# AlvinHon/ring-zk

Hardware: AMD Instinct MI355X
Metric: proofs/sec (commit+challenge+response+verify), N=1024, batch=4096; NTT GB/s vs HBM peak (higher is better)
Workload: dtype u32

## Files before the change

### ring_zk_amd/csrc/rzk_core.h

```cpp
#pragma once
#include <stdint.h>

#if defined(__HIPCC__)
#include <hip/hip_runtime.h>
#define RZK_HD __host__ __device__ __forceinline__
#else
#define RZK_HD inline
#endif

namespace rzk {

constexpr int kMaxPrimes = 3;
constexpr int kKeyImages = kMaxPrimes;
constexpr int kTableLog = 12;
constexpr int kTableLen = 1 << kTableLog;

constexpr uint32_t kPrimes[kMaxPrimes] = {1073692673u, 1073668097u, 1073651713u};
constexpr uint32_t kPrimeGenerators[kMaxPrimes] = {3u, 3u, 10u};

struct PrimeConsts {
  uint32_t p;
  uint32_t twop;
  uint32_t npinv;
  uint32_t r2;
// ... 189 lines not shown
RZK_HD void inv_phase1(uint32_t* x, const uint32_t* tw, const PrimeConsts& pc) {
  using G = Geo<LOGN, LL>;
#pragma unroll
  for (int s = G::LE - 1; s >= 0; --s) {
    const int half = G::E >> (s + 1);
#pragma unroll
    for (int e = 0; e < G::E; ++e) {
      if (e & half) continue;
      const uint32_t w = tw[(1 << s) + (e >> (G::LE - s))];
      bfly_inv(x[e], x[e + half], w, pc);
    }
  }
}

RZK_HD uint32_t lift(int32_t v, const PrimeConsts& pc) { return (uint32_t)v + pc.twop; }

RZK_HD uint32_t mac_add(uint32_t acc, uint32_t x, uint32_t k, const PrimeConsts& pc) {
  return csub(acc + mont_lazy(x, k, pc.p, pc.npinv), pc.twop);
}
RZK_HD uint32_t mac_sub(uint32_t acc, uint32_t x, uint32_t k, const PrimeConsts& pc) {
  return csub(acc + pc.twop - mont_lazy(x, k, pc.p, pc.npinv), pc.twop);
}

struct CrtConsts {
  uint32_t q, qinv;
  uint32_t qhalf;
  uint32_t inv01_r;
  uint32_t p0_mod_p2_r;
  uint32_t inv012_r;
  uint32_t c1;
  uint32_t c2;
  uint32_t pmodq[4];
  uint32_t half1;
  uint32_t half3_d2;
  uint64_t half2;
  uint64_t half3_lo;
  uint32_t hmod[4][4];
  uint32_t hmodq[4];
  uint32_t r2q;
  uint32_t r48q;
};

RZK_HD int64_t montq(uint32_t a, uint32_t c, const CrtConsts& C) {
  uint64_t t = (uint64_t)a * c;
  uint32_t m = (uint32_t)t * C.qinv;
  uint32_t h = (uint32_t)(((uint64_t)m * C.q) >> 32);
  return (int64_t)(uint32_t)(t >> 32) - (int64_t)h;
}
template <int ROUNDS>
RZK_HD int64_t center_rounds(int64_t s, const CrtConsts& C) {
  const int64_t q = C.q, h = C.qhalf;
#pragma unroll
  for (int i = 0; i < ROUNDS; ++i) {
    s = s > h ? s - q : s;
    s = s < -h ? s + q : s;
  }
  return s;
}
RZK_HD int64_t crt_center(uint32_t r0, uint32_t r1, uint32_t r2, int np, const PrimeConsts* pc,
                          const CrtConsts& C) {
  const uint32_t d0 = csub(r0, pc[0].p);
  int64_t s = d0;
  bool neg;
// ... 37 lines not shown
  const uint32_t d = a - b;
  return a < b ? d + q : d;
}
RZK_HD uint32_t montq_u(uint32_t a, uint32_t c, const CrtConsts& C) {
  const uint64_t t = (uint64_t)a * c;
  const uint32_t m = (uint32_t)t * C.qinv;
  const uint32_t h = (uint32_t)(((uint64_t)m * C.q) >> 32);
  const uint32_t hi = (uint32_t)(t >> 32);
  const uint32_t d = hi - h;
  return hi < h ? d + C.q : d;
}
RZK_HD uint32_t zq_from_centered(int32_t a, uint32_t q) { return (uint32_t)a + (a < 0 ? q : 0u); }
RZK_HD int64_t center_from_zq(uint32_t u, const CrtConsts& C) {
  const uint32_t lo = u > C.qhalf ? u - C.q : u;
  return (int64_t)(int32_t)lo;
}
RZK_HD uint32_t crt2_zq(uint32_t r1, uint32_t d0, const PrimeConsts* pc, const CrtConsts& C) {
  const uint32_t t1 = r1 + pc[1].twop - d0;
  const uint32_t d1 = csub(mont_lazy(t1, C.inv01_r, pc[1].p, pc[1].npinv), pc[1].p);
  const uint32_t va = addq(d0, montq_u(d1, C.c1, C), C.q);
  const uint64_t x01 = (uint64_t)d1 * pc[0].p + d0;
  return subq(va, x01 >= C.half2 ? C.pmodq[2] : 0u, C.q);
}
RZK_HD uint32_t crt_digit1(uint32_t r, uint32_t d0, int np, const PrimeConsts* pc, const CrtConsts& C) {
  const uint32_t a1 = csub(csub(r + C.hmod[np][1], pc[1].twop), pc[1].p);
  const uint32_t t1 = a1 + pc[1].p - csub(d0, pc[1].p);
  return csub(mont_lazy(t1, C.inv01_r, pc[1].p, pc[1].npinv), pc[1].p);
}
RZK_HD uint32_t crt_value01_modq(uint32_t d0, uint32_t d1, const CrtConsts& C) {
  return addq(d0, montq_u(d1, C.c1, C), C.q);
}
RZK_HD uint32_t crt_value01_modp2(uint32_t d0, uint32_t d1, const PrimeConsts* pc, const CrtConsts& C) {
  const uint32_t m1 = mont_lazy(d1, C.p0_mod_p2_r, pc[2].p, pc[2].npinv);
  return csub(csub(d0, pc[2].p) + m1, pc[2].twop);
}
RZK_HD void crt_fold1(uint32_t r, int np, const PrimeConsts* pc, const CrtConsts& C, uint32_t& stA,
                      uint32_t& stB) {
  const uint32_t d0 = stA;
  const uint32_t d1 = crt_digit1(r, d0, np, pc, C);
  stA = crt_value01_modq(d0, d1, C);
  if (np == 3) stB = crt_value01_modp2(d0, d1, pc, C);
}
RZK_HD void crt_fold2(uint32_t r, const PrimeConsts* pc, const CrtConsts& C, uint32_t& stA, uint32_t stB) {
  const uint32_t a2 = csub(csub(r + C.hmod[3][2], pc[2].twop), pc[2].p);
  const uint32_t t2 = a2 + pc[2].twop - stB;
  const uint32_t d2 = csub(mont_lazy(t2, C.inv012_r, pc[2].p, pc[2].npinv), pc[2].p);
// ... 132 lines not shown
```

### ring_zk_amd/csrc/rzk_ctx.cpp

```cpp
#include "rzk_ctx.h"

namespace rzk::api {

void wipe(void* p, size_t n) {
  volatile uint8_t* v = (volatile uint8_t*)p;
  for (size_t i = 0; i < n; ++i) v[i] = 0;
}

int fail(rzk_ctx* c, int code, const char* msg) {
  if (c) c->err = msg;
  return code;
}

LaunchCfg cfg_of(rzk_ctx* c) {
  (void)hipSetDevice(c->device);
  return LaunchCfg{(void*)c->stream, c->num_cus, c->pair_poly ? 1 : 0, c->unit_io ? 1 : 0, c->shift_bytes ? 1 : 0};
}

int arena_reserve(rzk_ctx* c, Arena& a, size_t bytes) {
  if (bytes <= a.cap) return RZK_OK;
  HIPCHK(c, hipStreamSynchronize(c->stream));
  if (a.p) HIPCHK(c, hipFree(a.p));
  a.p = nullptr;
  a.cap = 0;
// ... 52 lines not shown
  constexpr Knob(const char* n, bool rzk_ctx::*f, const char* w) : name(n), kind(Bool), b(f), what(w) {}
  constexpr Knob(const char* n, Kind k, int rzk_ctx::*f, const char* w) : name(n), kind(k), i(f), what(w) {}
  constexpr Knob(const char* n, uint32_t rzk_ctx::*f, const char* w) : name(n), kind(Uint), u(f), what(w) {}
  constexpr Knob(const char* n, double rzk_ctx::*f, const char* w) : name(n), kind(Double), d(f), what(w) {}
};
const Knob kKnobs[] = {
    {"RZK_GRID_CUS", Knob::Clamped, &rzk_ctx::num_cus, "testing: CU count behind every grid cap and scratch size, in [1, the device's]"},
    {"RZK_SLOT_SHARE_MIN", &rzk_ctx::slot_share_min, "shared-operand path from this ratio of operand transforms to distinct operands"},
    {"RZK_ROW_GROUPS", &rzk_ctx::use_groups, "0: no row groups"},
    {"RZK_GROUP_MAX", Knob::Clamped, &rzk_ctx::group_max, "rows per group of row_group_kernel, in [1, the compiled accumulators]"},
    {"RZK_SHIFT", &rzk_ctx::use_shift, "0: challenge products as transforms, not rotations"},
    {"RZK_SHIFT_BYTES", &rzk_ctx::shift_bytes, "0: rotations of short operands as words, not packed bytes"},
    {"RZK_SUM_D", Knob::Flag, &rzk_ctx::sum_d, "Sum proof: force a2.(sum_i g_i v_i - v') on (1) or off (0); unset: by cost"},
    {"RZK_DKEY", Knob::Int, &rzk_ctx::use_dkey, "multiplier images: 0 never, 1 from kDkeyMinUses rows per multiplier on, 2 always"},
    {"RZK_LIN_E", &rzk_ctx::lin_e, "0: Linear verifier in the reference's grouping"},
    {"RZK_OIMG", &rzk_ctx::use_oimg, "0: Sum proof without operand images"},
    {"RZK_PRESET_IN_KERNEL", &rzk_ctx::preset_in_kernel, "0: verdict flags always preset by a fill launch"},
    {"RZK_PAIRS", &rzk_ctx::use_pairs, "0: unit_kernel without row pairs"},
    {"RZK_UPT", &rzk_ctx::units_per_task, "units per task of unit_kernel (0: automatic)"},
    {"RZK_VEC_ROWS", &rzk_ctx::vec_rows, "0: vector x vector programs on unit_kernel, not row_kernel"},
    {"RZK_PAIR_POLY", &rzk_ctx::pair_poly, "0: one wavefront per polynomial at N = 2048"},
    {"RZK_UNIT_IO", &rzk_ctx::unit_io, "0 / 1: force unit_kernel / unit_io_kernel for key-product programs (default: N = 512 only)"},
    {"RZK_BLOCK_MIN_LOGN", &rzk_ctx::block_min_logn, "row blocks from this log2 N on (12: never)"},
};

void read_knobs(rzk_ctx* c) {
  for (const Knob& k : kKnobs) {
    const char* e = std::getenv(k.name);
    if (!e) continue;
    switch (k.kind) {
      case Knob::Bool: c->*k.b = std::atoi(e) != 0; break;
      case Knob::Flag: c->*k.i = std::atoi(e) != 0 ? 1 : 0; break;
      case Knob::Int: c->*k.i = std::atoi(e); break;
      case Knob::Uint: c->*k.u = (uint32_t)std::atoi(e); break;
      case Knob::Double: c->*k.d = std::atof(e); break;
      case Knob::Clamped:
        if (k.i == &rzk_ctx::num_cus) {
          const long v = std::strtol(e, nullptr, 10);
          c->num_cus = v < 1 ? 1 : (v < c->num_cus ? (int)v : c->num_cus);
        } else {
          const int g = std::atoi(e);
          if (g >= 1 && g <= group_accumulators(c->logn)) c->group_max = g;
        }
        break;
    }
  }
// ... 26 lines not shown
  c->r2q = (uint32_t)((((unsigned __int128)1) << 64) % (unsigned __int128)q);
  c->n = n;
  c->k = k;
  c->l = l;
  c->kappa = kappa;
  c->b = b;
  c->sigma = b * (11ull * kappa) * isqrt_u64((uint64_t)k * N);
  c->commit_bound = 4 * c->sigma * isqrt_u64(N);
  c->verify_bound = 2 * c->sigma * isqrt_u64(N);
  if (!host::make_crt_consts((uint64_t)q, c->hT.crt)) {
    delete c;
    return create_fail(RZK_E_UNSUPPORTED, "modulus must be odd and below 4 * the smallest auxiliary prime");
  }
  if ((de = hipSetDevice(device)) != hipSuccess) {
    delete c;
    return create_fail(RZK_E_HIP, std::string("hipSetDevice: ") + hipGetErrorString(de));
  }
  hipDeviceProp_t prop;
  if (hipGetDeviceProperties(&prop, device) == hipSuccess && prop.multiProcessorCount > 0)
    c->num_cus = prop.multiProcessorCount;
  c->group_max = group_max_for((int)c->logn);
  c->unit_io = c->logn == 9;
  read_knobs(c);
  if ((de = hipStreamCreateWithFlags(&c->own_stream, hipStreamNonBlocking)) != hipSuccess) {
    delete c;
    return create_fail(RZK_E_HIP, std::string("hipStreamCreate: ") + hipGetErrorString(de));
  }
  c->stream = c->own_stream;

  std::vector<uint32_t> all((size_t)2 * kMaxPrimes * kTableLen);
  for (int i = 0; i < kMaxPrimes; ++i) {
    std::vector<uint32_t> f, v;
    host::make_twiddles(i, f, v);
    std::memcpy(&all[(size_t)(2 * i) * kTableLen], f.data(), sizeof(uint32_t) * kTableLen);
    std::memcpy(&all[(size_t)(2 * i + 1) * kTableLen], v.data(), sizeof(uint32_t) * kTableLen);
    c->hT.pc[i] = host::make_prime_consts(i, N);
  }
  bool okk = hipMalloc((void**)&c->d_tw, all.size() * sizeof(uint32_t)) == hipSuccess &&
             hipMemcpy(c->d_tw, all.data(), all.size() * sizeof(uint32_t), hipMemcpyHostToDevice) == hipSuccess;
  c->hT.cap[0] = 0.0;
  for (int np = 1; np <= kMaxPrimes; ++np) c->hT.cap[np] = host::crt_capacity(np);
  okk = okk && (c->small || hipMalloc((void**)&c->d_row_scratch,
                                      row_scratch_words((int)c->logn, c->num_cus) * sizeof(uint32_t)) == hipSuccess);
  okk = okk && hipMalloc((void**)&c->dT, sizeof(DevTables)) == hipSuccess &&
        hipMemcpy(c->dT, &c->hT, sizeof(DevTables), hipMemcpyHostToDevice) == hipSuccess;
  okk = okk && hipMalloc((void**)&c->d_bad, sizeof(uint32_t)) == hipSuccess &&
// ... 167 lines not shown
```

### ring_zk_amd/csrc/rzk_ctx.h

```cpp
#pragma once
#include <hip/hip_runtime.h>

#include <cmath>
#include <cstddef>
#include <cstdio>
#include <cstdlib>
#include <cstring>
#include <map>
#include <memory>
#include <string>
#include <utility>
#include <vector>

#include "../../include/rzk.h"
#include "rzk_chacha.h"
#include "rzk_core.h"
#include "rzk_dev.h"
#include "rzk_dgauss.h"
#include "rzk_keccak.h"
#include "rzk_packed.h"
#include "rzk_plan.h"
#include "rzk_reject.h"
#include "rzk_tables.h"
#include "rzk_xof.h"
// ... 31 lines not shown
struct rzk_ctx {
  int device = 0;
  hipStream_t own_stream = nullptr;
  hipStream_t stream = nullptr;
  int num_cus = 256;
  int64_t q = 0;
  uint32_t N = 0, logn = 0, n = 0, k = 0, l = 0, kappa = 0;
  uint64_t b = 0;
  uint64_t sigma = 0, commit_bound = 0, verify_bound = 0;
  DevTables hT{};
  DevTables* dT = nullptr;
  uint32_t* d_tw = nullptr;
  uint32_t* d_row_scratch = nullptr;
  uint32_t* d_group_scratch = nullptr;
  uint32_t* d_block_scratch = nullptr;
  uint32_t block_min_logn = 11;
  bool use_groups = true;
  uint32_t units_per_task = 0;
  bool vec_rows = true;
  bool unit_io = false;
  bool pair_poly = true;
  bool trusted = false;
  bool use_pairs = true;
  int group_max = 1;
  bool use_shift = true;
  bool shift_bytes = true;
  int use_dkey = 1;
  Arena ws_dkey;
  const uint32_t* dkey_img = nullptr;
  const double* dkey_l2 = nullptr;
  uint32_t dkey_n = 0;
  bool use_oimg = true;
  Arena ws_oimg;
  Operands oimg_state{};
  uint32_t oimg_producer_op = 0xffu;
  bool lin_e = true;
  int sum_d = -1;
  bool preset_in_kernel = true;
  bool small = false;
  uint32_t r2q = 0;
  uint32_t* d_key_mont = nullptr;
  bool key_loaded = false;
  std::vector<uint8_t> key_class;
  std::vector<int32_t> key_entry;
  uint32_t n_general = 0;
  uint32_t* d_key_ntt = nullptr;
// ... 135 lines not shown
```

### ring_zk_amd/csrc/rzk_dev.h

```cpp
#pragma once
#include <stddef.h>
#include <stdint.h>

#include <string>

#include "rzk_core.h"
#include "rzk_packed.h"
#include "rzk_wire_walk.h"

namespace rzk {

struct DevTables {
  PrimeConsts pc[kMaxPrimes];
  CrtConsts crt;
  double cap[kMaxPrimes + 1];
};

#if defined(__HIPCC__)
template <class Tp>
__device__ __forceinline__ Tp table_load(const Tp* p) {
#if defined(__HIP_DEVICE_COMPILE__)
  typedef const Tp __attribute__((address_space(4))) * cptr_t;
  return *reinterpret_cast<cptr_t>(reinterpret_cast<uintptr_t>(p));
#else
  return *p;
#endif
}
#endif
constexpr int kMaxOperands = 12;
constexpr int kMaxRows = 48;
constexpr int kMaxTerms = 640;
constexpr int kMaxAdds = 128;

enum : uint8_t { TERM_KEY = 0, TERM_VEC = 1, TERM_SHIFT = 2, TERM_DKEY = 3, TERM_DD = 4, TERM_KIND_MASK = 0x3f };
enum : uint8_t { MODE_STORE = 0, MODE_ZERO = 1 };
constexpr uint8_t TERM_CHECK = 0x80;
constexpr uint8_t TERM_CHECK2 = 0x40;
constexpr uint8_t ADD_CHECK = 0x80;
// ... 12 lines not shown
  uint16_t off;
};
struct alignas(8) Row {
  uint16_t term0, nterms, add0, nadds;
  uint8_t out_op, mode;
  uint16_t out_off;
  uint16_t nshift, pad;
};
constexpr int kGroupMax = 4;
struct GroupDesc {
  uint16_t row0, count;
};
struct Program {
  uint32_t nrows, nterms, nadds, ngroups;
  GroupDesc groups[kMaxRows];
  Row rows[kMaxRows];
  Term terms[kMaxTerms];
  AddTerm adds[kMaxAdds];
};

enum : uint8_t { ITEM_KEY = 0, ITEM_VEC = 1 };
constexpr uint16_t kNoKey = 0xffff;
constexpr uint16_t kNoRow = 0xffff;
struct alignas(8) Item {
  uint8_t kind;
  uint8_t flags;
  uint8_t b_op, a_op;
  uint16_t b_off, a_off;
  uint16_t keyA, keyB;
  int8_t signA, signB;
  uint16_t pad;
};
struct alignas(8) Unit {
  uint16_t rowA, rowB;
  uint16_t item0, nitems;
};
struct WaveProgram {
  uint32_t nunits, nitems;
  Unit units[kMaxRows];
  Item items[kMaxTerms];
};

constexpr int kMaxSlots = 512;
struct SlotTable {
  uint32_t nslots, pad;
  uint16_t op[kMaxSlots], off[kMaxSlots];
// ... 167 lines not shown
```

### ring_zk_amd/csrc/rzk_plan.h

```cpp
#pragma once
#include <cstring>
#include <map>
#include <utility>

#include "rzk_dev.h"

namespace rzk {

static_assert(sizeof(Term) == 8 && sizeof(AddTerm) == 4 && sizeof(Row) == 16 && sizeof(Item) == 16 && sizeof(Unit) == 8,
              "program record sizes");
static_assert(offsetof(Program, rows) % 8 == 0 && offsetof(Program, terms) % 8 == 0 && offsetof(Program, adds) % 4 == 0 &&
                  offsetof(WaveProgram, units) % 8 == 0 && offsetof(WaveProgram, items) % 8 == 0,
              "program record alignment");

enum KeyClass : uint8_t { KC_ZERO = 0, KC_ONE = 1, KC_GENERAL = 2 };

enum ProgId : int {
  PG_MATVEC = 0,
  PG_POLYMUL,
  PG_CMUL,
  PG_OPEN_COMMIT,
  PG_RESPONSE,
  PG_A1_RELATION,
  PG_LIN_COMMIT2,
// ... 14 lines not shown
  PG_LIN_V2B,
};

constexpr uint32_t kDkeyVar = 0x10000u;
constexpr uint32_t kOimgVar = 0x20000u;
constexpr uint32_t kRecoverVar = 0x40000u;
inline bool recover_capable(int id) {
  return id == PG_A1_RELATION || id == PG_REL_ROT || id == PG_LIN_V1B || id == PG_LIN_V2B || id == PG_SUM_V3 || id == PG_SUM_V4;
}

constexpr int kPlanOk = 0, kPlanArg = -1, kPlanUnsupported = -4;

struct PlanEnv {
  uint32_t n, k, l, logn;
  bool small;
  bool rot;
  uint32_t block_min_logn;
  bool use_groups;
  int group_max;
  bool use_pairs;
  double slot_share_min;
  const uint8_t* key_class;
  const int32_t* key_entry;
};

struct PlanFacts {
  uint32_t nrows = 0;
  uint32_t nunits = 0;
  uint32_t work = 0;
  bool has_vec = false;
  uint32_t nslots = 0;
  uint32_t np_store = 0;
  uint32_t ngroups = 0;
  uint32_t nblocks = 0;
  bool has_dkey = false;
  bool has_dd = false;
  bool shift = false;
  bool has_shift = false;
  bool two_bit = false;
  uint16_t polys_in[kMaxOperands] = {};
  uint32_t polys_out = 0;
};

struct Plan {
  Program prog;
  WaveProgram wave;
// ... 370 lines not shown
  uint32_t ng = 0;
  for (uint32_t r = 0; r < p.nrows;) {
    uint32_t cnt = 1;
    const Row& r0 = p.rows[r];
    while (cnt < gmax && r + cnt < p.nrows) {
      const Row& rr = p.rows[r + cnt];
      bool same = rr.nterms == r0.nterms && r0.nterms > 0;
      for (uint32_t t = 0; same && t < r0.nterms; ++t) {
        const Term& a = p.terms[r0.term0 + t];
        const Term& b2 = p.terms[rr.term0 + t];
        same = a.b_op == b2.b_op && a.b_off == b2.b_off;
      }
      if (!same) break;
      ++cnt;
    }
    p.groups[ng].row0 = (uint16_t)r;
    p.groups[ng].count = (uint16_t)cnt;
    ++ng;
    r += cnt;
  }
  return ng * 2 <= p.nrows ? ng : 0;
}

inline uint32_t plan_units(const Program& p, bool use_pairs, WaveProgram& wp) {
  auto key_only = [&](const Row& rr) {
    for (uint32_t t = 0; t < rr.nterms; ++t)
      if (kind_of(p.terms[rr.term0 + t]) != TERM_KEY) return false;
    return true;
  };
  uint32_t work = 0;
  for (uint32_t r = 0; r < p.nrows;) {
    const Row& ra = p.rows[r];
    Unit& un = wp.units[wp.nunits++];
    un.rowA = (uint16_t)r;
    un.rowB = kNoRow;
    un.item0 = (uint16_t)wp.nitems;
    un.nitems = ra.nterms;
    for (uint32_t t = 0; t < ra.nterms; ++t) {
      const Term& tm = p.terms[ra.term0 + t];
      Item& im = wp.items[wp.nitems++];
      im.kind = kind_of(tm) == TERM_VEC ? ITEM_VEC : ITEM_KEY;
      im.flags = tm.kind & (TERM_CHECK | TERM_CHECK2);
      im.b_op = tm.b_op;
      im.b_off = tm.b_off;
      im.a_op = tm.a_op;
      im.a_off = tm.a_off;
      im.keyA = im.kind == ITEM_KEY ? tm.a_off : 0;
      im.keyB = kNoKey;
      im.signA = tm.sign;
      im.signB = 0;
    }
    uint32_t step = 1;
    if (use_pairs && r + 1 < p.nrows && ra.nterms >= 1 && ra.nshift == 0 && key_only(ra)) {
      const Row& rb = p.rows[r + 1];
      if (rb.nterms == 1 && rb.nshift == 0 && key_only(rb)) {
        const Term& tb = p.terms[rb.term0];
        const Term& ta = p.terms[ra.term0 + ra.nterms - 1];
        if (tb.b_op == ta.b_op && tb.b_off == ta.b_off) {
          Item& im = wp.items[wp.nitems - 1];
          im.keyB = tb.a_off;
          im.signB = tb.sign;
          im.flags |= tb.kind & (TERM_CHECK | TERM_CHECK2);
          un.rowB = (uint16_t)(r + 1);
          step = 2;
        }
      }
    }
    work += (un.nitems ? un.nitems : 1u) + (un.rowB != kNoRow ? 2u : 1u);
    r += step;
  }
  return work;
}

inline bool plan_slots(const Program& p, double share_min, SlotTable& st) {
  std::map<OpOff, uint32_t> index;
  bool fits = true;
  uint32_t transforms = 0;
  auto slot_of = [&](uint8_t op, uint16_t off) -> uint32_t {
    auto it = index.find({op, off});
    if (it != index.end()) return it->second;
    if (st.nslots >= (uint32_t)kMaxSlots) { fits = false; return 0; }
    const uint32_t sidx = st.nslots++;
    st.op[sidx] = op;
    st.off[sidx] = off;
    index[{op, off}] = sidx;
    return sidx;
  };
  for (uint32_t t = 0; t < p.nterms; ++t) {
    const Term& tm = p.terms[t];
    const uint32_t sb = slot_of(tm.b_op, tm.b_off);
// ... 48 lines not shown
  bool key_only = p.nterms > 0, all_sparse = p.nterms > 0;
  for (uint32_t t = 0; t < p.nterms; ++t) {
    const Term& tm = p.terms[t];
    const uint8_t kind = kind_of(tm);
    key_only = key_only && kind == TERM_KEY;
    all_sparse = all_sparse && tm.kind == TERM_VEC && ((pb.sparse_ops >> tm.a_op) & 1u);
    f.has_vec = f.has_vec || kind == TERM_VEC;
    f.has_shift = f.has_shift || kind == TERM_SHIFT;
    f.has_dd = f.has_dd || kind == TERM_DD;
    f.has_dkey = f.has_dkey || kind == TERM_DKEY || kind == TERM_DD;
  }
  f.shift = env.rot && pb.sparse_ops && all_sparse;
  f.two_bit = pb.two_bit;
  f.nrows = p.nrows;
  if (!env.small && env.logn >= 10 && env.logn >= env.block_min_logn && !f.shift && !f.has_shift && !f.two_bit &&
      !f.has_dkey && p.nterms > 0) {
    plan.use_blocks = plan_blocks(p, key_only, plan.blocks);
    if (plan.use_blocks) f.nblocks = plan.blocks.nblocks;
  }
  if (!env.small && env.use_groups && !f.shift && !f.two_bit && !f.nblocks && !f.has_dkey && key_only)
    p.ngroups = f.ngroups = plan_groups(p, (uint32_t)env.group_max);
  if (!env.small) {
    plan.use_wave = true;
    f.work = plan_units(p, env.use_pairs, plan.wave);
    f.nunits = plan.wave.nunits;
  }
  if (!env.small && env.slot_share_min > 0 && p.nterms > 0 && f.ngroups == 0 && !f.shift && !f.has_shift &&
      !f.two_bit && !f.nblocks && !f.has_dkey) {
    plan.use_slots = plan_slots(p, env.slot_share_min, plan.slots);
    if (plan.use_slots) {
      f.nslots = plan.slots.nslots;
      f.np_store = f.has_vec ? 3 : 2;
    }
  }
  count_traffic(p, f);
  return kPlanOk;
}

}
```

### ring_zk_amd/csrc/rzk_rowprog.h

```cpp
#pragma once
#include "rzk_wave.h"

namespace rzk {

__device__ __forceinline__ int32_t canon_lo(int64_t c, uint32_t qhalf, uint32_t& bad) {
  bad |= (uint32_t)(((uint64_t)c + qhalf) >> 32);
  return (int32_t)c;
}
__device__ __forceinline__ int32_t canon_lo_mx(int64_t c, uint32_t qhalf, uint32_t& bad, uint32_t& mx) {
  const uint64_t s = (uint64_t)c + qhalf;
  bad |= (uint32_t)(s >> 32);
  const uint32_t lo = (uint32_t)s;
  mx = lo > mx ? lo : mx;
  return (int32_t)c;
}
__device__ __forceinline__ void canon_pair(const longlong2 t, uint32_t qhalf, uint32_t& bad, uint32_t& mx, int32_t& lo0,
                                           int32_t& lo1) {
  lo0 = canon_lo_mx(t.x, qhalf, bad, mx);
  lo1 = canon_lo_mx(t.y, qhalf, bad, mx);
}
__device__ __forceinline__ bool canon_fail(uint32_t bad, uint32_t mx, uint32_t qhalf) {
  return __any((bad != 0) | (mx > 2u * qhalf)) != 0;
}
__device__ __forceinline__ void input_fault(const Operands& ops, uint8_t* flags, uint32_t bo, int lane) {
// ... 234 lines not shown
      for (int i = 0; i < H; ++i) {
        const int64_t c = p[i * S::LANES + lane];
        vh[i] = canon ? canon_lo_mx(c, qhalf, bad, mx) : (int32_t)c;
      }
    }
    if (measure) {
#pragma unroll
      for (int i = 0; i < H; ++i) {
        const uint32_t uu = (uint32_t)vh[i];
        const uint32_t vv = vh[i] < 0 ? 0u - uu : uu;
        maxabs = vv > maxabs ? vv : maxabs;
      }
    }
    int32_t* base = ext + S::lane_base(lane) + h * HOFF;
#pragma unroll
    for (int i = 0; i < H; ++i) {
      const int32_t a = shift_part(vh[i], part);
      base[S::N + S::off(i)] = a;
      base[S::off(i)] = -a;
    }
  }
}

template <int LOGN, bool PAIR, bool TO_MEM, class TM = WaveTeam>
__device__ __forceinline__ void shift_product(uint32_t* res, bool fresh, bool minus, const int32_t* a,
                                              const int64_t* __restrict__ pv, int lane_in, int32_t* ext,
                                              const DevTables& T, bool& fault, bool trusted) {
  constexpr int LL = TM::LL;
  int lane = lane_in;
  if (LL != 6) asm volatile("" : "+v"(lane));
  using S = ShiftGeo<LOGN, PAIR, LL>;
  constexpr int E = S::E;
  constexpr int HW = TO_MEM ? (LL == 6 ? kShiftHMem : kShiftHMemPair) : kShiftH;
  constexpr int H = HW < E ? HW : E;
  constexpr int NCH = E / H;
  constexpr bool LIST = LL != 6;
  const uint32_t q = T.crt.q, qhalf = T.crt.qhalf;
  uint32_t vbad = 0, vmx = 0, maxv = 0;
  TM::sync();
  shift_fill_from<LOGN, PAIR, LL>(pv, lane, ext, SHIFT_WHOLE, true, !trusted, qhalf, vbad, vmx, maxv);
  if (!trusted) fault = fault || canon_fail(vbad, vmx, qhalf);
  uint64_t suma = 0;
#pragma unroll
  for (int i = 0; i < E; ++i) {
    const uint32_t ua = (uint32_t)a[i];
    suma += a[i] < 0 ? 0u - ua : ua;
  }
  const double bound = (double)TM::sum_u56(suma) * (double)TM::max_u32(maxv);
  const int npass = __builtin_amdgcn_readfirstlane(bound < 4.0e18 ? 1 : 2);
  int32_t* list = ext + S::WORDS;
  uint32_t lbase = 0, ltotal = 1;
  if (LIST) {
    const uint32_t mine = shift_count_nonzeros<E>(a);
    const uint32_t w = (uint32_t)__builtin_amdgcn_readfirstlane(lane >> 6);
    if ((lane & 63) == 0) list[2 * kShiftListCap + w] = (int32_t)mine;
    TM::sync();
// ... 382 lines not shown
```

### ring_zk_amd/csrc/rzk_run.cpp

```cpp
#include "rzk_ctx.h"

namespace rzk::api {

bool shift_ok(const rzk_ctx* c) { return c->use_shift && !c->small && (c->logn <= 10 || c->pair_poly); }

namespace {

PlanEnv plan_env(const rzk_ctx* c) {
  return PlanEnv{c->n, c->k, c->l, c->logn, c->small, shift_ok(c), c->block_min_logn, c->use_groups, c->group_max,
                 c->use_pairs, c->slot_share_min, c->key_class.data(), c->key_entry.data()};
}

template <class T>
int upload(rzk_ctx* c, const T* host, T** dev) {
  HIPCHK(c, hipMalloc((void**)dev, sizeof(T)));
  HIPCHK(c, hipMemcpyAsync(*dev, host, sizeof(T), hipMemcpyHostToDevice, c->stream));
  HIPCHK(c, hipStreamSynchronize(c->stream));
  return RZK_OK;
}

void free_program(DevProg& dp) {
  if (dp.d) (void)hipFree(dp.d);
  if (dp.d_slots) (void)hipFree(dp.d_slots);
  if (dp.d_blocks) (void)hipFree(dp.d_blocks);
  if (dp.d_wp) (void)hipFree(dp.d_wp);
}

int get_program(rzk_ctx* c, int id, uint32_t var, DevProg& out) {
  const bool needs_key = !(id == PG_POLYMUL || id == PG_CMUL || id == PG_RESPONSE || id == PG_SUM_XP ||
                           id == PG_SUM_W2 || id == PG_REL_ROT);
  if (needs_key && !c->key_loaded) return fail(c, RZK_E_STATE, "commitment key not loaded");
  auto it = c->progs.find({id, var});
  if (it != c->progs.end()) {
// ... 286 lines not shown
```

### ring_zk_amd/csrc/rzk_tables.h

```cpp
#pragma once
#include <cstdint>
#include <vector>

#include "rzk_core.h"

namespace rzk {
namespace host {

typedef unsigned __int128 u128;

inline uint64_t mulmod(uint64_t a, uint64_t b, uint64_t m) { return (uint64_t)((u128)a * b % m); }
inline uint64_t powmod(uint64_t b, uint64_t e, uint64_t m) {
  uint64_t r = 1 % m;
  b %= m;
  while (e) {
    if (e & 1) r = mulmod(r, b, m);
    b = mulmod(b, b, m);
    e >>= 1;
  }
  return r;
}
inline uint64_t invmod_prime(uint64_t a, uint64_t p) { return powmod(a, p - 2, p); }
inline uint32_t inv_u32(uint32_t odd) {
  uint32_t x = odd;
// ... 60 lines not shown
  C.p0_mod_p2_r = to_mont(p0 % p2, (uint32_t)p2);
  C.inv012_r = to_mont(invmod_prime(mulmod(p0 % p2, p1 % p2, p2), p2), (uint32_t)p2);
  C.c1 = (uint32_t)(((u128)(p0 % q) << 32) % q);
  C.c2 = (uint32_t)(((u128)mulmod(p0 % q, p1 % q, q) << 32) % q);
  C.pmodq[0] = 1 % q;
  C.pmodq[1] = (uint32_t)(p0 % q);
  C.pmodq[2] = (uint32_t)mulmod(p0 % q, p1 % q, q);
  C.pmodq[3] = (uint32_t)mulmod(C.pmodq[2], p2 % q, q);
  C.half1 = (uint32_t)((p0 + 1) / 2);
  C.half2 = (p0 * p1 + 1) / 2;
  const u128 P3 = (u128)p0 * p1 * p2;
  const u128 h3 = (P3 + 1) / 2;
  C.half3_d2 = (uint32_t)(h3 / (p0 * p1));
  C.half3_lo = (uint64_t)(h3 % (p0 * p1));
  for (int np = 0; np <= kMaxPrimes; ++np) {
    u128 P = 1;
    for (int i = 0; i < np; ++i) P *= kPrimes[i];
    const u128 H = (P - 1) / 2;
    for (int i = 0; i < 4; ++i) C.hmod[np][i] = i < kMaxPrimes ? (uint32_t)(H % kPrimes[i]) : 0;
    C.hmodq[np] = (uint32_t)(H % q);
  }
  C.r2q = (uint32_t)((((u128)1) << 64) % q);
  C.r48q = (uint32_t)((((u128)1) << 48) % q);
  return true;
}

inline double crt_capacity(int np) {
  long double P = 1;
  for (int i = 0; i < np; ++i) P *= (long double)kPrimes[i];
  return (double)((P - 1) / 2 * (1.0L - 1e-12L));
}

}
}
```

### ring_zk_amd/csrc/rzk_unit.h

```cpp
#pragma once
#include "rzk_rowprog.h"

namespace rzk {

constexpr int kScratchLines = 6;
#ifndef RZK_STAMPS
#define RZK_STAMPS 0
#endif
#if RZK_STAMPS
#define RZK_T0() const uint64_t t_sec0 = __builtin_amdgcn_s_memtime()
#define RZK_T1(acc) acc += __builtin_amdgcn_s_memtime() - t_sec0
#else
#define RZK_T0() do { } while (0)
#define RZK_T1(acc) do { } while (0)
#endif

__device__ __forceinline__ void set_priority_level(uint32_t level) {
  if (level == 0) __builtin_amdgcn_s_setprio(3);
  else if (level == 1) __builtin_amdgcn_s_setprio(2);
  else if (level == 2) __builtin_amdgcn_s_setprio(1);
  else __builtin_amdgcn_s_setprio(0);
}
__device__ __forceinline__ void set_progress_priority(uint32_t done, uint32_t total) {
  set_priority_level(__builtin_amdgcn_readfirstlane(total ? (done * 4u) / total : 0u));
// ... 69 lines not shown
  }
  if (!EARLY && pi == 2) {
#pragma unroll
    for (int g = 0; g < E / 4; ++g) sb[g] = B4[G::own4(li, g)];
  }
  if (pi == 0) {
    if (np == 1) {
#pragma unroll
      for (int e = 0; e < E; ++e) acc[e] = crt1_zq(acc[e], T.pc, T.crt);
      return true;
    }
    if (np == 2) {
#pragma unroll
      for (int e = 0; e < E; ++e) acc[e] = crt2_digit0(acc[e], T.pc);
    } else {
#pragma unroll
      for (int e = 0; e < E; ++e) acc[e] = crt_fold0(acc[e], np, T.pc, T.crt);
    }
#pragma unroll
    for (int g = 0; g < E / 4; ++g) A4[G::own4(li, g)] = make_uint4(acc[4 * g], acc[4 * g + 1], acc[4 * g + 2], acc[4 * g + 3]);
    return false;
  }
  if (pi == 1 && np == 2) {
#pragma unroll
    for (int g = 0; g < E / 4; ++g) {
      const uint4 dv = sa[g];
      const uint32_t d0[4] = {dv.x, dv.y, dv.z, dv.w};
#pragma unroll
      for (int i = 0; i < 4; ++i) acc[4 * g + i] = crt2_zq(acc[4 * g + i], d0[i], T.pc, T.crt);
    }
    return true;
  }
  if (pi == 1) {
#pragma unroll
    for (int g = 0; g < E / 4; ++g) {
      const uint4 dv = sa[g];
      const uint32_t d0[4] = {dv.x, dv.y, dv.z, dv.w};
      uint32_t va[4], vb[4];
#pragma unroll
      for (int i = 0; i < 4; ++i) {
        const uint32_t d1 = crt_digit1(acc[4 * g + i], d0[i], np, T.pc, T.crt);
        va[i] = crt_value01_modq(d0[i], d1, T.crt);
        vb[i] = crt_value01_modp2(d0[i], d1, T.pc, T.crt);
      }
      A4[G::own4(li, g)] = make_uint4(va[0], va[1], va[2], va[3]);
      B4[G::own4(li, g)] = make_uint4(vb[0], vb[1], vb[2], vb[3]);
// ... 91 lines not shown
#define RZK_STEP_PRIORITY()                             \
  do {                                                  \
    set_progress_priority(work_done, work_total);       \
    ++work_done;                                        \
  } while (0)

  for (uint32_t task = first_task; task < ntasks; task += gridDim.x * WPB) {
    const uint32_t b = task / tasks_per_entry;
    const uint32_t u0 = (task - b * tasks_per_entry) * units_per_task;
    const uint32_t u1 = u0 + units_per_task < nunits ? u0 + units_per_task : nunits;
    const uint32_t bo = ops.group > 1 ? b / ops.group : b;
    if (ops.preset) {
      if (lane == 0) flags[bo] = (uint8_t)ops.preset;
      if (TM::LL != 6) TM::sync();
    }
#pragma unroll 1
    for (uint32_t ui = u0; ui < u1; ++ui) {
      const Unit un = table_load(&wp->units[ui]);
      const Row rowA = table_load(&prog->rows[un.rowA]);
      const bool pair = un.rowB != kNoRow;
      const uint32_t un_items = un.nitems;
      const bool null_unit = un_items == 0;
      const bool has_shift = HAS_SHIFT && rowA.nshift > 0;
      if (has_shift) {
        bool fault = false;
        RZK_T0();
#pragma unroll 1
        for (uint32_t t = 0; t < rowA.nshift; ++t) {
          const Term tm = table_load(&prog->terms[rowA.term0 + rowA.nterms + t]);
          const int64_t* __restrict__ pa = operand_ptr(ops, tm.a_op, tm.a_off, b, bo, N);
          int32_t a[E];
          if (trusted) {
#pragma unroll
            for (int e = 0; e < E; ++e) a[e] = (int32_t)pa[G::j_p1(lane, e)];
          } else {
            uint32_t abad = 0, amx = 0;
#pragma unroll
            for (int e = 0; e < E; ++e) a[e] = canon_lo_mx(pa[G::j_p1(lane, e)], qhalf, abad, amx);
            fault = fault || canon_fail(abad, amx, qhalf);
          }
          shift_product<LOGN, false, true, TM>(st_sh, t == 0, tm.sign < 0, a, operand_ptr(ops, tm.b_op, tm.b_off, b, bo, N), lane,
                                           reinterpret_cast<int32_t*>(lds), T, fault, trusted);
        }
        if (fault) input_fault(ops, flags, bo, lane);
        TM::sync();
        RZK_T1(t_rot);
      }
// ... 9 lines not shown
#pragma unroll 1
        for (uint32_t it = 0; it < nit; ++it) {
          const bool last = it + 1 == nit;
          RZK_STEP_PRIORITY();
          int ln = lane;
          RZK_OPAQUE(ln);
          uint32_t acc[E];
#pragma unroll
          for (int c = 0; c < E; ++c) acc[c] = 0;
          if (!null_unit) {
            const Item im = table_load(&wp->items[un.item0 + it]);
            uint32_t x[E];
            float nb = 0.f;
            bool below = true;
            const bool chk = first && (im.flags & (TERM_CHECK | TERM_CHECK2));
            {
              RZK_T0();
              load_lift<LOGN, TM>(x, operand_ptr(ops, im.b_op, im.b_off, b, bo, N), ln, pc, first, nb, chk, ops.norm_limit, below, qhalf,
                              trusted, fault);
              RZK_T1(t_load);
            }
            if (chk && !below && (lane & 63) == 0) fail_check(flags + bo, ops.pad != 0, (im.flags & TERM_CHECK2) != 0);
            const bool vec = HAS_VEC && im.kind == ITEM_VEC;
            constexpr bool EARLY = E <= 16 && !HAS_VEC;
            uint32_t kreg[E];
            const uint4* __restrict__ kpA = reinterpret_cast<const uint4*>(key_ntt + ((size_t)im.keyA * kKeyImages + pi) * N);
            if (EARLY && !vec && im.keyA != kNoKey) {
#pragma unroll
              for (int g = 0; g < E / 4; ++g) {
                const uint4 kv = kpA[G::key4(ln, g)];
                kreg[4 * g] = kv.x, kreg[4 * g + 1] = kv.y, kreg[4 * g + 2] = kv.z, kreg[4 * g + 3] = kv.w;
              }
            }
            {
              RZK_T0();
              wave_fwd<LOGN, TM>(x, ln, lds, twf, pc);
              RZK_T1(t_fwd);
            }
            if (!EARLY && !vec && im.keyA != kNoKey) {
#pragma unroll
              for (int g = 0; g < E / 4; ++g) {
                const uint4 kv = kpA[G::key4(ln, g)];
                kreg[4 * g] = kv.x, kreg[4 * g + 1] = kv.y, kreg[4 * g + 2] = kv.z, kreg[4 * g + 3] = kv.w;
              }
            }
            uint32_t xb[E];
            if (vec) {
#pragma unroll
              for (int c = 0; c < E; ++c) xb[c] = csub(mont_lazy(x[c], pc.ninv_r2, pc.p, pc.npinv), pc.p);
              float na = 0.f;
              bool unused_below = true;
              load_lift<LOGN, TM>(x, operand_ptr(ops, im.a_op, im.a_off, b, bo, N), ln, pc, first, na, false, 0, unused_below, qhalf,
                              trusted, fault);
              wave_fwd<LOGN, TM>(x, ln, lds, twf, pc);
              if (first) boundA = bound_fma(na, nb, boundA);
            } else if (first) {
              if (im.keyA != kNoKey) boundA = bound_fma((float)key_l2[im.keyA], nb, boundA);
              if (pair && im.keyB != kNoKey) boundB = bound_fma((float)key_l2[im.keyB], nb, boundB);
            }
            const bool feedsA = vec || im.keyA != kNoKey;
            if (!last) {
              RZK_T0();
              if (vec) mac_park<LOGN, false, TM>(x, xb, im.signA < 0, P4, ln, it == 0, pc);
              else if (feedsA) mac_park<LOGN, false, TM>(x, kreg, im.signA < 0, P4, ln, it == 0, pc);
              RZK_T1(t_mac);
              continue;
            }
            RZK_T0();
            if (fault) input_fault(ops, flags, bo, lane);
            if (first) np = primes_for(boundA > boundB ? boundA : boundB, T);
#pragma unroll
            for (int c = 0; c < E; ++c) acc[c] = x[c];
            if (vec) {
              mac_park<LOGN, true, TM>(acc, xb, im.signA < 0, P4, ln, it == 0, pc);
            } else if (feedsA) {
              mac_park<LOGN, true, TM>(acc, kreg, im.signA < 0, P4, ln, it == 0, pc);
            } else {
#pragma unroll
              for (int g = 0; g < E / 4; ++g) {
                const uint4 v = P4[G::own4(ln, g)];
                acc[4 * g] = v.x, acc[4 * g + 1] = v.y, acc[4 * g + 2] = v.z, acc[4 * g + 3] = v.w;
              }
            }
            if (pair) {
              const uint4* __restrict__ kb = reinterpret_cast<const uint4*>(key_ntt + ((size_t)im.keyB * kKeyImages + pi) * N);
              uint32_t kbr[E];
#pragma unroll
              for (int g = 0; g < E / 4; ++g) {
                const uint4 kv = kb[G::key4(ln, g)];
                kbr[4 * g] = kv.x, kbr[4 * g + 1] = kv.y, kbr[4 * g + 2] = kv.z, kbr[4 * g + 3] = kv.w;
              }
              mac_park<LOGN, false, TM>(x, kbr, im.signB < 0, P4, ln, true, pc);
            }
            RZK_T1(t_mac);
          }
#pragma unroll 1
          for (uint32_t r = 0; r < (pair ? 2u : 1u); ++r) {
            if (r == 1) {
#pragma unroll
              for (int g = 0; g < E / 4; ++g) {
                const uint4 v = P4[G::own4(ln, g)];
                acc[4 * g] = v.x, acc[4 * g + 1] = v.y, acc[4 * g + 2] = v.z, acc[4 * g + 3] = v.w;
              }
            }
            bool done = true;
            RZK_STEP_PRIORITY();
            if (!null_unit) {
              RZK_T0();
              done = inverse_fold_global<LOGN, OPQ, TM>(pi, np, acc, lane, lds, twf + kTableLen, pc, st + (size_t)(2 * r) * N,
                                                    st + (size_t)(2 * r + 1) * N, T);
              RZK_T1(t_inv);
            }
            if (done) {
              RZK_T0();
              finish_row<LOGN, 16, TM>(acc, prog, table_load(&prog->rows[r ? un.rowB : un.rowA]), ops, b, bo, lane, T, flags,
                               (has_shift && r == 0) ? st_sh : nullptr);
              RZK_T1(t_fin);
            }
          }
        }
      }
    }
  }
#undef RZK_STEP_PRIORITY
#if RZK_STAMPS
  if (lane == 0) {
    const uint64_t stamp1 = __builtin_amdgcn_s_memrealtime();
    uint32_t hwid;
    asm volatile("s_getreg_b32 %0, hwreg(HW_REG_HW_ID)" : "=s"(hwid));
    uint32_t xcc;
    asm volatile("s_getreg_b32 %0, hwreg(HW_REG_XCC_ID)" : "=s"(xcc));
    uint32_t* o = st + kScratchLines * N;
    o[0] = (uint32_t)stamp0, o[1] = (uint32_t)(stamp0 >> 32), o[2] = (uint32_t)stamp1, o[3] = (uint32_t)(stamp1 >> 32);
    o[4] = hwid, o[5] = xcc, o[6] = blockIdx.x, o[7] = wave;
    const uint64_t cyc1 = __builtin_amdgcn_s_memtime();
    o[8] = (uint32_t)(cyc1 - cyc0);
    o[9] = (uint32_t)t_load, o[10] = (uint32_t)t_fwd, o[11] = (uint32_t)t_mac, o[12] = (uint32_t)t_inv, o[13] = (uint32_t)t_fin, o[14] = (uint32_t)t_rot;
  }
#endif
// ... 233 lines not shown
        int li = lane;
        RZK_OPAQUE(li);
        const bool have = r == 1 || haveA;
        uint32_t u[E];
        if (!have) {
#pragma unroll
          for (int e = 0; e < E; ++e) u[e] = 0;
        } else {
          uint32_t a[E];
          if (r == 0) unpark<LOGN, TM>(a, const_cast<const uint4*>(P4), li);
          else if (B0L) unpark<LOGN, TM>(a, const_cast<const uint4*>(PB0), li);
          else unpark<LOGN, TM>(a, reinterpret_cast<const uint4*>(st + 1 * N), li);
          RZK_STEP_PRIORITY();
          RZK_OPAQUE(li);
          wave_inv<LOGN, TM>(a, li, lds, tw_all + (size_t)(2 * 0 + 1) * kTableLen, T.pc[0]);
          if (np == 2) {
#pragma unroll
            for (int e = 0; e < E; ++e) u[e] = crt2_digit0(a[e], T.pc);
            if (P1L && r == 0) unpark<LOGN, TM>(a, const_cast<const uint4*>(P41), li);
            else unpark<LOGN, TM>(a, reinterpret_cast<const uint4*>(st + (r == 0 ? 0 : 2) * N), li);
            RZK_STEP_PRIORITY();
            RZK_OPAQUE(li);
            wave_inv<LOGN, TM>(a, li, lds, tw_all + (size_t)(2 * 1 + 1) * kTableLen, T.pc[1]);
#pragma unroll
            for (int e = 0; e < E; ++e) u[e] = crt2_zq(a[e], u[e], T.pc, T.crt);
          } else {
            uint32_t wb[E];
#pragma unroll
            for (int e = 0; e < E; ++e) u[e] = crt_fold0(a[e], 3, T.pc, T.crt);
            if (P1L && r == 0) unpark<LOGN, TM>(a, const_cast<const uint4*>(P41), li);
            else unpark<LOGN, TM>(a, reinterpret_cast<const uint4*>(st + (r == 0 ? 0 : 2) * N), li);
            RZK_STEP_PRIORITY();
            RZK_OPAQUE(li);
            wave_inv<LOGN, TM>(a, li, lds, tw_all + (size_t)(2 * 1 + 1) * kTableLen, T.pc[1]);
#pragma unroll
            for (int e = 0; e < E; ++e) {
              wb[e] = 0;
              crt_fold1(a[e], 3, T.pc, T.crt, u[e], wb[e]);
            }
            unpark<LOGN, TM>(a, reinterpret_cast<const uint4*>(st + (r == 0 ? 3 : 5) * N), li);
            RZK_STEP_PRIORITY();
            RZK_OPAQUE(li);
            wave_inv<LOGN, TM>(a, li, lds, tw_all + (size_t)(2 * 2 + 1) * kTableLen, T.pc[2]);
#pragma unroll
            for (int e = 0; e < E; ++e) {
              crt_fold2(a[e], T.pc, T.crt, u[e], wb[e]);
              u[e] = crt_finish_zq(u[e], 3, T.crt);
            }
// ... 27 lines not shown
```

Before: 15.50 million.

## Fuse two-key row products, shorten two-prime CRT, and apply rotations after inverse

Adds three default-on options in unit_kernel. First, a two-product key row parks its raw transform and then reduces both products with a single Montgomery reduction of the 64-bit sum (dot2_lazy). Second, two-prime CRT reconstruction folds the centering correction and both digits into one mod-q Montgomery reduction (crt2_zq_short). Third, rotation terms are applied to the accumulator after the inverse transform, skipping the scratch-line round trip. The aim is fewer modular reductions and less global scratch traffic, at the cost of more code paths and 64-bit sums whose overflow safety rests on the lazy bounds.

```diff
diff --git a/ring_zk_amd/csrc/rzk_core.h b/ring_zk_amd/csrc/rzk_core.h
--- a/ring_zk_amd/csrc/rzk_core.h
+++ b/ring_zk_amd/csrc/rzk_core.h
@@ -235,6 +235,13 @@
   return csub(acc + pc.twop - mont_lazy(x, k, pc.p, pc.npinv), pc.twop);
 }
 
+RZK_HD uint32_t dot2_lazy(uint32_t x1, uint32_t k1, uint32_t x2, uint32_t k2, const PrimeConsts& pc) {
+  const uint64_t t = (uint64_t)x1 * k1 + (uint64_t)x2 * k2;
+  const uint32_t m = (uint32_t)t * pc.npinv;
+  const uint64_t u = (uint64_t)m * pc.p + t;
+  return csub((uint32_t)(u >> 32), pc.twop);
+}
+
 struct CrtConsts {
   uint32_t q, qinv;
   uint32_t qhalf;
@@ -252,6 +259,9 @@
   uint32_t hmodq[4];
   uint32_t r2q;
   uint32_t r48q;
+  uint32_t half2_d1, half2_d0;
+  uint32_t r1q;
+  uint32_t knq;
 };
 
 RZK_HD int64_t montq(uint32_t a, uint32_t c, const CrtConsts& C) {
@@ -335,6 +345,18 @@
   const uint64_t x01 = (uint64_t)d1 * pc[0].p + d0;
   return subq(va, x01 >= C.half2 ? C.pmodq[2] : 0u, C.q);
 }
+RZK_HD uint32_t crt2_zq_short(uint32_t r1, uint32_t d0, const PrimeConsts* pc, const CrtConsts& C) {
+  const uint32_t t1 = r1 + pc[1].twop - d0;
+  const uint32_t d1 = csub(mont_lazy(t1, C.inv01_r, pc[1].p, pc[1].npinv), pc[1].p);
+  const bool neg = d1 >= C.half2_d1 + (d0 < C.half2_d0 ? 1u : 0u);
+  uint64_t t = (uint64_t)d1 * C.c1 + (uint64_t)(neg ? C.knq : 0u);
+  t += (uint64_t)d0 * C.r1q;
+  const uint32_t m = (uint32_t)t * C.qinv;
+  const uint32_t h = (uint32_t)(((uint64_t)m * C.q) >> 32);
+  uint32_t d;
+  const bool borrow = __builtin_sub_overflow((uint32_t)(t >> 32), h, &d);
+  return borrow ? d + C.q : d;
+}
 RZK_HD uint32_t crt_digit1(uint32_t r, uint32_t d0, int np, const PrimeConsts* pc, const CrtConsts& C) {
   const uint32_t a1 = csub(csub(r + C.hmod[np][1], pc[1].twop), pc[1].p);
   const uint32_t t1 = a1 + pc[1].p - csub(d0, pc[1].p);
diff --git a/ring_zk_amd/csrc/rzk_ctx.cpp b/ring_zk_amd/csrc/rzk_ctx.cpp
--- a/ring_zk_amd/csrc/rzk_ctx.cpp
+++ b/ring_zk_amd/csrc/rzk_ctx.cpp
@@ -98,6 +98,9 @@
     {"RZK_PAIR_POLY", &rzk_ctx::pair_poly, "0: one wavefront per polynomial at N = 2048"},
     {"RZK_UNIT_IO", &rzk_ctx::unit_io, "0 / 1: force unit_kernel / unit_io_kernel for key-product programs (default: N = 512 only)"},
     {"RZK_BLOCK_MIN_LOGN", &rzk_ctx::block_min_logn, "row blocks from this log2 N on (12: never)"},
+    {"RZK_ROT_LAST", &rzk_ctx::rot_last, "0: unit_kernel evaluates every row's rotation terms first, through its scratch line"},
+    {"RZK_DOT2", &rzk_ctx::dot2, "0: unit_kernel reduces each of a two-product row's products on its own"},
+    {"RZK_CRT2_SHORT", &rzk_ctx::crt2_short, "0: two-prime reconstruction with two reductions mod q (crt2_zq)"},
 };
 
 void read_knobs(rzk_ctx* c) {
@@ -170,6 +173,7 @@
   c->group_max = group_max_for((int)c->logn);
   c->unit_io = c->logn == 9;
   read_knobs(c);
+  c->hT.diet = (c->rot_last ? DIET_ROT_LAST : 0u) | (c->crt2_short ? DIET_CRT2 : 0u);
   if ((de = hipStreamCreateWithFlags(&c->own_stream, hipStreamNonBlocking)) != hipSuccess) {
     delete c;
     return create_fail(RZK_E_HIP, std::string("hipStreamCreate: ") + hipGetErrorString(de));
diff --git a/ring_zk_amd/csrc/rzk_ctx.h b/ring_zk_amd/csrc/rzk_ctx.h
--- a/ring_zk_amd/csrc/rzk_ctx.h
+++ b/ring_zk_amd/csrc/rzk_ctx.h
@@ -77,6 +77,9 @@
   bool pair_poly = true;
   bool trusted = false;
   bool use_pairs = true;
+  bool rot_last = true;
+  bool dot2 = true;
+  bool crt2_short = true;
   int group_max = 1;
   bool use_shift = true;
   bool shift_bytes = true;
diff --git a/ring_zk_amd/csrc/rzk_dev.h b/ring_zk_amd/csrc/rzk_dev.h
--- a/ring_zk_amd/csrc/rzk_dev.h
+++ b/ring_zk_amd/csrc/rzk_dev.h
@@ -14,6 +14,12 @@
   PrimeConsts pc[kMaxPrimes];
   CrtConsts crt;
   double cap[kMaxPrimes + 1];
+  uint32_t diet;
+  uint32_t pad;
+};
+enum : uint32_t {
+  DIET_ROT_LAST = 1,
+  DIET_CRT2 = 2,
 };
 
 #if defined(__HIPCC__)
@@ -72,6 +78,7 @@
 enum : uint8_t { ITEM_KEY = 0, ITEM_VEC = 1 };
 constexpr uint16_t kNoKey = 0xffff;
 constexpr uint16_t kNoRow = 0xffff;
+constexpr uint8_t ITEM_DOT2 = 0x01;
 struct alignas(8) Item {
   uint8_t kind;
   uint8_t flags;
diff --git a/ring_zk_amd/csrc/rzk_plan.h b/ring_zk_amd/csrc/rzk_plan.h
--- a/ring_zk_amd/csrc/rzk_plan.h
+++ b/ring_zk_amd/csrc/rzk_plan.h
@@ -60,6 +60,7 @@
   double slot_share_min;
   const uint8_t* key_class;
   const int32_t* key_entry;
+  bool dot2 = false;
 };
 
 struct PlanFacts {
@@ -476,7 +477,7 @@
   return ng * 2 <= p.nrows ? ng : 0;
 }
 
-inline uint32_t plan_units(const Program& p, bool use_pairs, WaveProgram& wp) {
+inline uint32_t plan_units(const Program& p, bool use_pairs, WaveProgram& wp, bool dot2 = false) {
   auto key_only = [&](const Row& rr) {
     for (uint32_t t = 0; t < rr.nterms; ++t)
       if (kind_of(p.terms[rr.term0 + t]) != TERM_KEY) return false;
@@ -520,6 +521,11 @@
         }
       }
     }
+    if (dot2 && un.nitems == 2) {
+      Item* two = &wp.items[un.item0];
+      if (two[0].kind == ITEM_KEY && two[1].kind == ITEM_KEY && two[0].keyA != kNoKey && two[1].keyA != kNoKey)
+        two[0].flags |= ITEM_DOT2, two[1].flags |= ITEM_DOT2;
+    }
     work += (un.nitems ? un.nitems : 1u) + (un.rowB != kNoRow ? 2u : 1u);
     r += step;
   }
@@ -614,7 +620,7 @@
     p.ngroups = f.ngroups = plan_groups(p, (uint32_t)env.group_max);
   if (!env.small) {
     plan.use_wave = true;
-    f.work = plan_units(p, env.use_pairs, plan.wave);
+    f.work = plan_units(p, env.use_pairs, plan.wave, env.dot2);
     f.nunits = plan.wave.nunits;
   }
   if (!env.small && env.slot_share_min > 0 && p.nterms > 0 && f.ngroups == 0 && !f.shift && !f.has_shift &&
diff --git a/ring_zk_amd/csrc/rzk_rowprog.h b/ring_zk_amd/csrc/rzk_rowprog.h
--- a/ring_zk_amd/csrc/rzk_rowprog.h
+++ b/ring_zk_amd/csrc/rzk_rowprog.h
@@ -280,7 +280,7 @@
   }
 }
 
-template <int LOGN, bool PAIR, bool TO_MEM, class TM = WaveTeam>
+template <int LOGN, bool PAIR, bool TO_MEM, class TM = WaveTeam, int HREG = kShiftH>
 __device__ __forceinline__ void shift_product(uint32_t* res, bool fresh, bool minus, const int32_t* a,
                                               const int64_t* __restrict__ pv, int lane_in, int32_t* ext,
                                               const DevTables& T, bool& fault, bool trusted) {
@@ -289,7 +289,7 @@
   if (LL != 6) asm volatile("" : "+v"(lane));
   using S = ShiftGeo<LOGN, PAIR, LL>;
   constexpr int E = S::E;
-  constexpr int HW = TO_MEM ? (LL == 6 ? kShiftHMem : kShiftHMemPair) : kShiftH;
+  constexpr int HW = TO_MEM ? (LL == 6 ? kShiftHMem : kShiftHMemPair) : HREG;
   constexpr int H = HW < E ? HW : E;
   constexpr int NCH = E / H;
   constexpr bool LIST = LL != 6;
diff --git a/ring_zk_amd/csrc/rzk_run.cpp b/ring_zk_amd/csrc/rzk_run.cpp
--- a/ring_zk_amd/csrc/rzk_run.cpp
+++ b/ring_zk_amd/csrc/rzk_run.cpp
@@ -8,7 +8,7 @@
 
 PlanEnv plan_env(const rzk_ctx* c) {
   return PlanEnv{c->n, c->k, c->l, c->logn, c->small, shift_ok(c), c->block_min_logn, c->use_groups, c->group_max,
-                 c->use_pairs, c->slot_share_min, c->key_class.data(), c->key_entry.data()};
+                 c->use_pairs, c->slot_share_min, c->key_class.data(), c->key_entry.data(), c->dot2};
 }
 
 template <class T>
diff --git a/ring_zk_amd/csrc/rzk_tables.h b/ring_zk_amd/csrc/rzk_tables.h
--- a/ring_zk_amd/csrc/rzk_tables.h
+++ b/ring_zk_amd/csrc/rzk_tables.h
@@ -106,6 +106,10 @@
   }
   C.r2q = (uint32_t)((((u128)1) << 64) % q);
   C.r48q = (uint32_t)((((u128)1) << 48) % q);
+  C.half2_d1 = (uint32_t)(C.half2 / p0);
+  C.half2_d0 = (uint32_t)(C.half2 % p0);
+  C.r1q = (uint32_t)((((u128)1) << 32) % q);
+  C.knq = (uint32_t)(((u128)((q - C.pmodq[2]) % q) << 32) % q);
   return true;
 }
 
diff --git a/ring_zk_amd/csrc/rzk_unit.h b/ring_zk_amd/csrc/rzk_unit.h
--- a/ring_zk_amd/csrc/rzk_unit.h
+++ b/ring_zk_amd/csrc/rzk_unit.h
@@ -115,6 +115,16 @@
     return false;
   }
   if (pi == 1 && np == 2) {
+    if (T.diet & DIET_CRT2) {
+#pragma unroll
+      for (int g = 0; g < E / 4; ++g) {
+        const uint4 dv = sa[g];
+        const uint32_t d0[4] = {dv.x, dv.y, dv.z, dv.w};
+#pragma unroll
+        for (int i = 0; i < 4; ++i) acc[4 * g + i] = crt2_zq_short(acc[4 * g + i], d0[i], T.pc, T.crt);
+      }
+      return true;
+    }
 #pragma unroll
     for (int g = 0; g < E / 4; ++g) {
       const uint4 dv = sa[g];
@@ -252,7 +262,8 @@
       const uint32_t un_items = un.nitems;
       const bool null_unit = un_items == 0;
       const bool has_shift = HAS_SHIFT && rowA.nshift > 0;
-      if (has_shift) {
+      const bool rot_last = has_shift && TM::LL == 6 && E <= 16 && !pair && (T.diet & DIET_ROT_LAST) != 0;
+      if (has_shift && !rot_last) {
         bool fault = false;
         RZK_T0();
 #pragma unroll 1
@@ -308,10 +319,12 @@
             }
             if (chk && !below && (lane & 63) == 0) fail_check(flags + bo, ops.pad != 0, (im.flags & TERM_CHECK2) != 0);
             const bool vec = HAS_VEC && im.kind == ITEM_VEC;
+            const bool dot2 = !HAS_VEC && TM::LL == 6 && E <= 16 && (im.flags & ITEM_DOT2) != 0;
             constexpr bool EARLY = E <= 16 && !HAS_VEC;
             uint32_t kreg[E];
             const uint4* __restrict__ kpA = reinterpret_cast<const uint4*>(key_ntt + ((size_t)im.keyA * kKeyImages + pi) * N);
-            if (EARLY && !vec && im.keyA != kNoKey) {
+            const bool want_key = !vec && im.keyA != kNoKey && !(dot2 && !last);
+            if (EARLY && want_key) {
 #pragma unroll
               for (int g = 0; g < E / 4; ++g) {
                 const uint4 kv = kpA[G::key4(ln, g)];
@@ -323,7 +336,7 @@
               wave_fwd<LOGN, TM>(x, ln, lds, twf, pc);
               RZK_T1(t_fwd);
             }
-            if (!EARLY && !vec && im.keyA != kNoKey) {
+            if (!EARLY && want_key) {
 #pragma unroll
               for (int g = 0; g < E / 4; ++g) {
                 const uint4 kv = kpA[G::key4(ln, g)];
@@ -347,8 +360,14 @@
             const bool feedsA = vec || im.keyA != kNoKey;
             if (!last) {
               RZK_T0();
-              if (vec) mac_park<LOGN, false, TM>(x, xb, im.signA < 0, P4, ln, it == 0, pc);
-              else if (feedsA) mac_park<LOGN, false, TM>(x, kreg, im.signA < 0, P4, ln, it == 0, pc);
+              if (vec) {
+                mac_park<LOGN, false, TM>(x, xb, im.signA < 0, P4, ln, it == 0, pc);
+              } else if (dot2) {
+#pragma unroll
+                for (int g = 0; g < E / 4; ++g) P4[G::own4(ln, g)] = make_uint4(x[4 * g], x[4 * g + 1], x[4 * g + 2], x[4 * g + 3]);
+              } else if (feedsA) {
+                mac_park<LOGN, false, TM>(x, kreg, im.signA < 0, P4, ln, it == 0, pc);
+              }
               RZK_T1(t_mac);
               continue;
             }
@@ -359,6 +378,30 @@
             for (int c = 0; c < E; ++c) acc[c] = x[c];
             if (vec) {
               mac_park<LOGN, true, TM>(acc, xb, im.signA < 0, P4, ln, it == 0, pc);
+            } else if (dot2) {
+              const Item im0 = table_load(&wp->items[un.item0]);
+              const uint4* __restrict__ kp1 = reinterpret_cast<const uint4*>(key_ntt + ((size_t)im0.keyA * kKeyImages + pi) * N);
+              uint32_t k1[E];
+#pragma unroll
+              for (int g = 0; g < E / 4; ++g) {
+                const uint4 kv = kp1[G::key4(ln, g)];
+                k1[4 * g] = kv.x, k1[4 * g + 1] = kv.y, k1[4 * g + 2] = kv.z, k1[4 * g + 3] = kv.w;
+              }
+              if (im.signA < 0) {
+#pragma unroll
+                for (int c = 0; c < E; ++c) kreg[c] = pc.p - kreg[c];
+              }
+              if (im0.signA < 0) {
+#pragma unroll
+                for (int c = 0; c < E; ++c) k1[c] = pc.p - k1[c];
+              }
+#pragma unroll
+              for (int g = 0; g < E / 4; ++g) {
+                const uint4 v = P4[G::own4(ln, g)];
+                const uint32_t x1[4] = {v.x, v.y, v.z, v.w};
+#pragma unroll
+                for (int i = 0; i < 4; ++i) acc[4 * g + i] = dot2_lazy(x1[i], k1[4 * g + i], x[4 * g + i], kreg[4 * g + i], pc);
+              }
             } else if (feedsA) {
               mac_park<LOGN, true, TM>(acc, kreg, im.signA < 0, P4, ln, it == 0, pc);
             } else {
@@ -397,10 +440,34 @@
                                                     st + (size_t)(2 * r + 1) * N, T);
               RZK_T1(t_inv);
             }
+            if (done && rot_last) {
+              RZK_T0();
+              bool sfault = false;
+#pragma unroll 1
+              for (uint32_t t = 0; t < rowA.nshift; ++t) {
+                const Term tm = table_load(&prog->terms[rowA.term0 + rowA.nterms + t]);
+                const int64_t* __restrict__ pa = operand_ptr(ops, tm.a_op, tm.a_off, b, bo, N);
+                int32_t a[E];
+                if (trusted) {
+#pragma unroll
+                  for (int e = 0; e < E; ++e) a[e] = (int32_t)pa[G::j_p1(lane, e)];
+                } else {
+                  uint32_t abad = 0, amx = 0;
+#pragma unroll
+                  for (int e = 0; e < E; ++e) a[e] = canon_lo_mx(pa[G::j_p1(lane, e)], qhalf, abad, amx);
+                  sfault = sfault || canon_fail(abad, amx, qhalf);
+                }
+                shift_product<LOGN, false, false, TM, kShiftHMem>(acc, false, tm.sign < 0, a, operand_ptr(ops, tm.b_op, tm.b_off, b, bo, N), lane,
+                                                  reinterpret_cast<int32_t*>(lds), T, sfault, trusted);
+              }
+              if (sfault) input_fault(ops, flags, bo, lane);
+              TM::sync();
+              RZK_T1(t_rot);
+            }
             if (done) {
               RZK_T0();
               finish_row<LOGN, 16, TM>(acc, prog, table_load(&prog->rows[r ? un.rowB : un.rowA]), ops, b, bo, lane, T, flags,
-                               (has_shift && r == 0) ? st_sh : nullptr);
+                               (has_shift && !rot_last && r == 0) ? st_sh : nullptr);
               RZK_T1(t_fin);
             }
           }
@@ -680,8 +747,13 @@
             RZK_STEP_PRIORITY();
             RZK_OPAQUE(li);
             wave_inv<LOGN, TM>(a, li, lds, tw_all + (size_t)(2 * 1 + 1) * kTableLen, T.pc[1]);
-#pragma unroll
-            for (int e = 0; e < E; ++e) u[e] = crt2_zq(a[e], u[e], T.pc, T.crt);
+            if (T.diet & DIET_CRT2) {
+#pragma unroll
+              for (int e = 0; e < E; ++e) u[e] = crt2_zq_short(a[e], u[e], T.pc, T.crt);
+            } else {
+#pragma unroll
+              for (int e = 0; e < E; ++e) u[e] = crt2_zq(a[e], u[e], T.pc, T.crt);
+            }
           } else {
             uint32_t wb[E];
 #pragma unroll
```

New measurement: 15.75 million (median of 6 runs). 1.6% higher.
